# hiimmuc/SpeakerVerification

Hardware: AMD Instinct MI355X
Metric: embeddings/sec (2 s @16 kHz) (higher is better)
Workload: dtype bf16

## Files before the change

### speakerverification_amd/csrc/api_ecapa.hip

```cpp
#include <algorithm>

#include "handle.h"

namespace svhip {

namespace {

struct EcapaState : ModelState {
    ConvLayer blocks0, mfa, asp_tdnn, asp_conv;
    ConvLayer tdnn1[3], tdnn2[3], res2[3][7];
    LinearLayer se1[3], se2[3], asp_ctx, fc;
    float* se2T[3] = {};
    void *se1_bf[3] = {}, *se2T_bf[3] = {};
    float *aspbn_scale = nullptr, *aspbn_shift = nullptr;

    bool xin_ready = false;
    bool x0_is_s32 = false;
    bool cat_f32_stale = false;
    bool h2_is_s32 = false;
    bool h1_split = false;
    void* cat_s32 = nullptr;
    void* h2_s32 = nullptr;
    void* u_s32[2] = {};
    void* X0 = nullptr;
// ... 31 lines not shown
    auto tdnn = [&](const std::string& p, int64_t cin, int64_t cout, int64_t k) {
        spec[p + ".conv.conv.weight"] = {cout, cin, k}; spec[p + ".conv.conv.bias"] = {cout};
        spec_bn(spec, p + ".norm.norm", cout);
    };
    if (c.input_norm) { spec["instance_norm.weight"] = {nm}; spec["instance_norm.bias"] = {nm}; }
    tdnn("blocks.0", nm, C, ECAPA_K[0]);
    for (int i = 1; i <= 3; ++i) {
        const std::string p = "blocks." + std::to_string(i);
        tdnn(p + ".tdnn1", C, C, 1);
        for (int j = 0; j < 7; ++j) tdnn(p + ".res2net_block.blocks." + std::to_string(j), C / 8, C / 8, ECAPA_K[i]);
        tdnn(p + ".tdnn2", C, C, 1);
        spec[p + ".se_block.conv1.conv.weight"] = {128, C, 1}; spec[p + ".se_block.conv1.conv.bias"] = {128};
        spec[p + ".se_block.conv2.conv.weight"] = {C, 128, 1}; spec[p + ".se_block.conv2.conv.bias"] = {C};
    }
    tdnn("mfa", C3, C3, 1);
    tdnn("asp.tdnn", 3 * C3, 128, 1);
    spec["asp.conv.conv.weight"] = {C3, 128, 1}; spec["asp.conv.conv.bias"] = {C3};
    spec_bn(spec, "asp_bn.norm", 2 * C3);
    spec["fc.conv.weight"] = {(int64_t)c.embed_dim, 2 * C3, 1}; spec["fc.conv.bias"] = {(int64_t)c.embed_dim};
}

static int make_tdnn(svhip_handle* h, ConvLayer& L, const std::string& p, int dil) {
    return make_conv(h, L, p + ".conv.conv.weight", p + ".conv.conv.bias", p + ".norm.norm", dil);
}

int ecapa_finalize(svhip_handle* h) {
    auto& s = S(h);
    const int C = h->cfg.channels, C3 = 3 * C;
    int rc;
    if ((rc = make_tdnn(h, s.blocks0, "blocks.0", ECAPA_D[0]))) return rc;
    for (int i = 1; i <= 3; ++i) {
        const std::string p = "blocks." + std::to_string(i);
        if ((rc = make_tdnn(h, s.tdnn1[i - 1], p + ".tdnn1", 1))) return rc;
        for (int j = 0; j < 7; ++j)
            if ((rc = make_tdnn(h, s.res2[i - 1][j], p + ".res2net_block.blocks." + std::to_string(j), ECAPA_D[i]))) return rc;
        if ((rc = make_tdnn(h, s.tdnn2[i - 1], p + ".tdnn2", 1))) return rc;
        if ((rc = make_linear(h, s.se1[i - 1], p + ".se_block.conv1.conv.weight", p + ".se_block.conv1.conv.bias"))) return rc;
        if ((rc = make_linear(h, s.se2[i - 1], p + ".se_block.conv2.conv.weight", p + ".se_block.conv2.conv.bias"))) return rc;
        {
            const HostTensor* w2 = getw(h, p + ".se_block.conv2.conv.weight");
            std::vector<float> t((size_t)128 * C);
            for (int c = 0; c < C; ++c)
                for (int n = 0; n < 128; ++n) t[(size_t)n * C + c] = w2->data[(size_t)c * 128 + n];
            if ((rc = dev_upload(h, &s.se2T[i - 1], t))) return rc;
            if (h->bf16) {
                const HostTensor* w1 = getw(h, p + ".se_block.conv1.conv.weight");
                if ((rc = upload_h16(h, w1->data, &s.se1_bf[i - 1])) || (rc = upload_h16(h, t, &s.se2T_bf[i - 1]))) return rc;
            }
        }
    }
    if ((rc = make_tdnn(h, s.mfa, "mfa", 1))) return rc;
    if ((rc = make_conv(h, s.asp_tdnn, "asp.tdnn.conv.conv.weight", "", "asp.tdnn.norm.norm", 1, 0, C3))) return rc;
    if ((rc = make_linear(h, s.asp_ctx, "asp.tdnn.conv.conv.weight", "asp.tdnn.conv.conv.bias", C3, 3 * C3))) return rc;
    if ((rc = make_conv(h, s.asp_conv, "asp.conv.conv.weight", "asp.conv.conv.bias", "", 1))) return rc;
    if ((rc = make_bn(h, "asp_bn.norm", 2 * C3, &s.aspbn_scale, &s.aspbn_shift))) return rc;
    if ((rc = make_linear(h, s.fc, "fc.conv.weight", "fc.conv.bias"))) return rc;
    if (h->cfg.input_norm) {
        const HostTensor *w = getw(h, "instance_norm.weight"), *b = getw(h, "instance_norm.bias");
        if (!w || !b) SV_FAIL(h, SVHIP_ERR_MISSING, "missing instance_norm tensors");
        if ((rc = dev_upload(h, &h->in_w, w->data))) return rc;
        if ((rc = dev_upload(h, &h->in_b, b->data))) return rc;
    }
    const double T = h->T;
    double f = T * s.blocks0.flops_per_row + T * s.mfa.flops_per_row + T * s.asp_conv.flops_per_row;
    f += T * 2.0 * 128 * (3.0 * C3);
    for (int i = 0; i < 3; ++i) {
        f += T * (s.tdnn1[i].flops_per_row + s.tdnn2[i].flops_per_row);
        for (int j = 0; j < 7; ++j) f += T * s.res2[i][j].flops_per_row;
// ... 149 lines not shown
                                    h->x3 ? h->d_status : nullptr, h->host_flag_dev, (b0_cv && xscale) ? 3.0e38f : 65504.0f);
         }))) return rc;
    if (b0_cv) {
        if (xscale && (rc = run(h, "in_scale", 0, [&]() {
                 return launch_in_scale(static_cast<const float*>(p.X_in), (int64_t)M * c.n_mels, reinterpret_cast<uint32_t*>(xscale + 4), xscale, p.st, L.cv_wscale);
             }))) return rc;
        if ((rc = run(h, "split_s32", 0, [&]() { return launch_split_s32(static_cast<const float*>(p.X_in), c.n_mels, h->s32_buf, M, L.cv_cin, p.st, L.cv_cin, c.n_mels, xscale); }))) return rc;
        if ((rc = run(h, "gemm_pw3cv", (double)M * L.flops_per_row, [&]() { return launch_gemm_pw3cv(q, p.st); }))) return rc;
        p.x0_s32 = q.y_s32 != 0;
    } else {
        GemmParams g = conv_params(h, L, p.X_in, c.n_mels, p.X0, C, M, T);
        g.act1 = ACT_GELU;
        if ((rc = conv_gemm(h, L, g))) return rc;
    }
    s.x0_is_s32 = p.x0_s32;
    p.xin = p.x0_s32 ? nullptr : p.X0;
    p.xin32 = p.x0_s32 ? p.X0 : nullptr;
    p.ldin = p.ldin32 = C;
    return SVHIP_OK;
}

static int ec_res2(EcPass& p, int i, EcRes2 route, bool tdnn1_side) {
    svhip_handle* h = p.h;
    auto& s = p.s;
    const int T = h->T, M = p.M, C = h->cfg.channels, C8 = C / 8, e = h->esz;
    const bool bf = h->bf16;
    int rc;
    if (route == RES2_CHAIN) {
        Res2Params rp;
        rp.H1 = p.H1; rp.H2 = p.H2; rp.ld = C; rp.T = T; rp.dil = s.res2[i][0].dil; rp.Kp = s.res2[i][0].Kp;
        rp.slices = h->opt.r2_slices >= 0 ? std::max(1, h->opt.r2_slices) : res2net_chain_slices(p.B, C, T, rp.dil, h->num_cu);
        double fl = 0;
        for (int j = 0; j < 7; ++j) {
            rp.W[j] = s.res2[i][j].W; rp.bias[j] = s.res2[i][j].bias;
            rp.scale[j] = s.res2[i][j].scale; rp.shift[j] = s.res2[i][j].shift;
            fl += (double)M * s.res2[i][j].flops_per_row;
        }
        return run(h, rp.slices > 1 ? "res2net_slices" : "res2net_chain", fl, [&]() { return launch_res2net_chain(rp, p.B, C, p.st); });
    }
    if (route == RES2_LAYERS) {
        if ((rc = run(h, "copy_cols", 0, [&]() { return launch_copy_cols(p.H1, C, p.H2, C, bf, M, C8, p.st); }))) return rc;
        for (int j = 1; j < 8; ++j) {
            GemmParams q = conv_params(h, s.res2[i][j - 1], off(p.H1, (size_t)j * C8, e), C, off(p.H2, (size_t)j * C8, e), C, M, T);
            q.act1 = ACT_RELU;
            q.A2 = j >= 2 ? off(p.H2, (size_t)(j - 1) * C8, e) : nullptr; q.lda2 = C;
            if ((rc = conv_gemm(h, s.res2[i][j - 1], q))) return rc;
        }
        return SVHIP_OK;
    }
    if (!tdnn1_side) {
        if ((rc = run(h, "split_s32", 0, [&]() { return launch_split_s32(static_cast<const float*>(p.H1), C, p.h2s, M, C8, p.st, C); }))) return rc;
        if ((rc = run(h, "split_s32", 0, [&]() { return launch_split_s32(static_cast<const float*>(p.H1) + C8, C, p.us[0], M, C8, p.st, C8); }))) return rc;
    }
    for (int j = 1; j < 8; ++j) {
        const GemmParams q = ec_r2_step_params(p, i, j);
        if ((rc = run(h, route == RES2_STEP ? "r2_step" : "gemm_pw3r2", (double)M * s.res2[i][j - 1].flops_per_row, [&]() {
                 return route == RES2_STEP ? launch_r2_step(q, p.st) : launch_gemm_pw3r2(q, p.st);
             }))) return rc;
    }
    return SVHIP_OK;
}

static int ec_block(EcPass& p, int i) {
    svhip_handle* h = p.h;
    auto& s = p.s;
    const int T = h->T, B = p.B, C = h->cfg.channels, C3 = 3 * C, C8 = C / 8, e = h->esz;
    const bool bf = h->bf16;
// ... 286 lines not shown
```

### speakerverification_amd/csrc/api_weights.hip

```cpp
#include <algorithm>
#include <cmath>
#include <cstring>

#include "handle.h"

namespace svhip {

static inline uint16_t f32_to_f16_rne(float f) {
    const _Float16 hv = static_cast<_Float16>(f);
    uint16_t u;
    memcpy(&u, &hv, 2);
    return u;
}

uint16_t f32_to_bf16_rne(float f) {
    uint32_t u;
    memcpy(&u, &f, 4);
    if ((u & 0x7fffffffu) > 0x7f800000u) return (uint16_t)((u >> 16) | 0x40);
    u += 0x7fffu + ((u >> 16) & 1u);
    return (uint16_t)(u >> 16);
}

uint32_t x3_split_word(float v) {
#ifdef SVHIP_X3_BF16
    const uint16_t hi = f32_to_bf16_rne(v);
    uint32_t hu = (uint32_t)hi << 16;
    float hf; memcpy(&hf, &hu, 4);
    return hu | f32_to_bf16_rne(v - hf);
#else
    const _Float16 h = static_cast<_Float16>(v);
    const _Float16 l = static_cast<_Float16>(v - static_cast<float>(h));
    uint16_t hb, lb;
    memcpy(&hb, &h, 2); memcpy(&lb, &l, 2);
    return ((uint32_t)hb << 16) | lb;
#endif
}

// ... 231 lines not shown
                    for (int k = 0; k < L.K; ++k) { const float a = std::fabs(packed[(size_t)n * L.Kp + k]); if (std::isfinite(a) && a > wmax) wmax = a; }
                float sw = 1.0f;
                if (wmax > 0.0f && !(wmax >= 0x1p-8f && wmax < 0x1p13f)) { int e2; (void)std::frexp(wmax, &e2); sw = std::ldexp(1.0f, 7 - e2); }
                L.cv_wscale = sw;
                std::vector<uint16_t> s32((size_t)N * kcv * 2, 0);
                for (int n = 0; n < N; ++n)
                    for (int t = 0; t < taps; ++t)
                        for (int c = 0; c < cin; ++c) {
                            const uint32_t wv = sw == 1.0f ? ws[(size_t)n * L.Kp + t * cin + c] : x3_split_word(packed[(size_t)n * L.Kp + t * cin + c] * sw);
                            const int k = t * ccv + c;
                            const size_t o = (size_t)n * kcv * 2 + (size_t)(k >> 5) * 64 + (k & 31);
                            s32[o] = (uint16_t)(wv >> 16);
                            s32[o + 32] = (uint16_t)(wv & 0xffffu);
                        }
                uint16_t* dcv;
                if ((rc = dev_upload(h, &dcv, s32))) return rc;
                L.Wcv = dcv; L.cv_cin = ccv; L.cv_Kp = kcv;
            }
        }
    }
    if (bias && (rc = dev_upload(h, &L.bias, *bias))) return rc;
    return SVHIP_OK;
}

int make_conv(svhip_handle* h, ConvLayer& L, const std::string& wname, const std::string& bname, const std::string& bnname, int dil,
              int c_lo, int c_hi, bool rn_s32) {
    const HostTensor *w, *b = nullptr;
    int rc;
    if ((rc = needw(h, wname, w)) || (!bname.empty() && (rc = needw(h, bname, b)))) return rc;
    if ((rc = make_conv(h, L, *w, b ? &b->data : nullptr, dil, c_lo, c_hi, rn_s32))) return rc;
    return bnname.empty() ? SVHIP_OK : make_bn(h, bnname, L.N, &L.scale, &L.shift);
}

int make_linear(svhip_handle* h, LinearLayer& L, const std::string& wname, const std::string& bname, int c_lo, int c_hi) {
    const HostTensor *w, *b = nullptr;
    int rc;
    if ((rc = needw(h, wname, w))) return rc;
    const int N = (int)w->shape[0], Kfull = (int)w->shape[1];
    if (c_hi < 0) c_hi = Kfull;
    L.N = N; L.K = c_hi - c_lo;
    std::vector<float> m((size_t)N * L.K);
    for (int n = 0; n < N; ++n)
        for (int k = 0; k < L.K; ++k) m[(size_t)n * L.K + k] = w->data[(size_t)n * Kfull + c_lo + k];
    if ((rc = dev_upload(h, &L.W, m))) return rc;
    if (!bname.empty() && ((rc = needw(h, bname, b)) || (rc = dev_upload(h, &L.bias, b->data)))) return rc;
    return SVHIP_OK;
}

int upload_f32(svhip_handle* h, const std::string& name, float** dst) {
    const HostTensor* t;
    int rc = needw(h, name, t);
    return rc ? rc : dev_upload(h, dst, t->data);
}

int upload_h16(svhip_handle* h, const std::vector<float>& m, void** dst) {
    std::vector<uint16_t> v(m.size());
    for (size_t i = 0; i < m.size(); ++i) v[i] = f32_to_bf16_rne(m[i]);
    uint16_t* d;
    int rc = dev_upload(h, &d, v);
    *dst = d;
    return rc;
}

int actbuf(svhip_handle* h, void** dst, size_t elems) {
    char* p = nullptr;
    int rc = dev_alloc(h, &p, elems * h->esz + 256);
// ... 34 lines not shown
```

### speakerverification_amd/csrc/handle.h

```cpp
#pragma once
#include "../../include/svhip.h"

#include <hip/hip_runtime.h>

#include <cstdio>
#include <initializer_list>
#include <map>
#include <memory>
#include <string>
#include <vector>

#include "common.h"
#include "kernels.h"

namespace svhip {

struct HostTensor {
    std::vector<float> data;
    std::vector<int64_t> shape;
    int64_t numel() const { int64_t n = 1; for (auto s : shape) n *= s; return n; }
};

struct ConvLayer {
    int N = 0, K = 0, Kp = 0, Np = 0, taps = 1, dil = 1, cin = 0;
    void* W = nullptr;
    void* Wsplit = nullptr;
    float cv_wscale = 1.0f;
    void* Wcv = nullptr;
    int cv_cin = 0, cv_Kp = 0;
    void* Ws32 = nullptr;
    float* bias = nullptr;
    float* scale = nullptr;
    float* shift = nullptr;
    double flops_per_row = 0;
};

struct LinearLayer {
    int N = 0, K = 0;
    float* W = nullptr;
    float* bias = nullptr;
};

struct ModelState { virtual ~ModelState() = default; };
struct TailedBuf { const char* base; size_t bytes; };

constexpr int RAG_LEVELS = 7;

struct ProfEntry { std::string name; double ms = 0; int64_t launches = 0; double flops = 0; };
struct PendingEvent { hipEvent_t e0, e1; int entry; };

}

struct svhip_handle {
    svhip_config cfg{};
    hipStream_t stream = nullptr;
    bool own_stream = false;
    hipStream_t cur = nullptr;
    hipStream_t lane_stream[4] = {nullptr, nullptr, nullptr, nullptr};
// ... 141 lines not shown
        pe.e1 = prof_event(h);
        (void)hipEventRecord(pe.e0, h->cur);
    }
    hipError_t e = launch();
    if (e != hipSuccess) SV_FAIL(h, SVHIP_ERR_HIP, "launch %s failed: %s", label, hipGetErrorString(e));
    if (prof) {
        (void)hipEventRecord(pe.e1, h->cur);
        h->prof_entries[pe.entry].launches += 1;
        h->prof_entries[pe.entry].flops += flops;
        h->ev_pending.push_back(pe);
        if (h->ev_pending.size() >= 8192) prof_collect(h);
    }
    return SVHIP_OK;
}

inline void* off(void* base, size_t elems, int esz) { return reinterpret_cast<char*>(base) + elems * esz; }
inline const void* off(const void* base, size_t elems, int esz) { return reinterpret_cast<const char*>(base) + elems * esz; }

using WeightSpec = std::map<std::string, std::vector<int64_t>>;
int build_fbank_tables(svhip_handle* h);
int alloc_workspace(svhip_handle* h);
uint16_t f32_to_bf16_rne(float f);
uint32_t x3_split_word(float v);
uint16_t to_h16(const svhip_handle* h, float f);
const HostTensor* getw(svhip_handle* h, const std::string& name);
int needw(svhip_handle* h, const std::string& name, const HostTensor*& t);
void spec_bn(WeightSpec& spec, const std::string& p, int64_t n);
int bn_fold(svhip_handle* h, const std::string& p, int n, std::vector<double>& s, std::vector<double>& t);
int make_bn(svhip_handle* h, const std::string& p, int n, float** scale, float** shift);
int make_conv(svhip_handle* h, ConvLayer& L, const HostTensor& w, const std::vector<float>* bias, int dil, int c_lo = 0, int c_hi = -1,
              bool rn_s32 = false);
int make_conv(svhip_handle* h, ConvLayer& L, const std::string& wname, const std::string& bname, const std::string& bnname, int dil,
              int c_lo = 0, int c_hi = -1, bool rn_s32 = false);
int make_linear(svhip_handle* h, LinearLayer& L, const std::string& wname, const std::string& bname, int c_lo = 0, int c_hi = -1);
int upload_f32(svhip_handle* h, const std::string& name, float** dst);
int upload_h16(svhip_handle* h, const std::vector<float>& m, void** dst);
int actbuf(svhip_handle* h, void** dst, size_t elems);

struct StageView { const void* src; size_t rows, cols, ld; bool f32; };
using CheckFn = int(const svhip_config& c, const char*& err);
using SpecFn = void(const svhip_config& c, WeightSpec& spec);
using HandleFn = int(svhip_handle* h);
using EmbedFn = int(svhip_handle* h, const float* in, int B);
using StageFn = int(svhip_handle* h, const std::string& name, bool fill, StageView& v);
using RaggedCheckFn = int(const svhip_config& c, const int32_t* lengths, int n, bool is_wave, std::string& err);
using RaggedEmbedFn = int(svhip_handle* h, const float* in, bool in_host, bool is_wave, const int64_t* in_off, const int32_t* lengths, int n);
struct ModelOps {
    int model;
    CheckFn* check;
    SpecFn* spec;
    HandleFn *finalize, *alloc;
    EmbedFn *embed_wave, *embed_feat;
    StageFn* stage;
    int max_lanes;
    const char* optional_prefix;
    RaggedCheckFn* ragged_check;
    RaggedEmbedFn* embed_ragged;
};
int unknown_stage(svhip_handle* h, const std::string& name);

struct KeptStages {
    struct Kept { void* buf = nullptr; size_t rows = 0, cols = 0; bool f32 = false; uint64_t epoch = 0; int utts = 0; bool packed = false; size_t cap = 0; };
    std::map<std::string, Kept> kept;
    uint64_t epoch = 0;
};
enum { KEEP_DT, KEEP_F32, KEEP_S32 };
// ... 63 lines not shown
```

### speakerverification_amd/csrc/kernels.h

```cpp
#pragma once
#include <hip/hip_runtime.h>
#include <stdint.h>

#include <atomic>

#include "common.h"

namespace svhip {

struct DeviceOnce {
    std::atomic<uint64_t> mask{0};
    bool done(int dev) const { return dev >= 0 && dev < 64 && ((mask.load(std::memory_order_acquire) >> dev) & 1u); }
    void mark(int dev) { if (dev >= 0 && dev < 64) mask.fetch_or(1ull << dev, std::memory_order_release); }
};
inline hipError_t set_max_dynamic_lds(DeviceOnce& once, const void* fn, int bytes) {
    int dev = -1;
    hipError_t e = hipGetDevice(&dev);
    if (e != hipSuccess) return e;
    if (once.done(dev)) return hipSuccess;
    e = hipFuncSetAttribute(fn, hipFuncAttributeMaxDynamicSharedMemorySize, bytes);
    if (e == hipSuccess) once.mark(dev);
    return e;
}

// ... 72 lines not shown
hipError_t launch_rn_step(const GemmParams& p, int mode, hipStream_t stream);
bool gemm_pw3cv_supported(const GemmParams& p);
hipError_t launch_gemm_pw3cv(const GemmParams& p, hipStream_t stream);
bool gemm_n128_supported(const GemmParams& p);
hipError_t launch_gemm_n128(const GemmParams& p, hipStream_t stream);
bool gemm_pw3cv16_supported(const GemmParams& p);
hipError_t launch_gemm_pw3cv16(const GemmParams& p, hipStream_t stream);
bool gemm_pw3r2_supported(const GemmParams& p);
hipError_t launch_gemm_pw3r2(const GemmParams& p, hipStream_t stream);
hipError_t launch_split_s32(const float* src, int ld, void* dst, int64_t M, int K, hipStream_t stream, int ldd = 0, int kvalid = 0,
                            const float* scale = nullptr);
hipError_t launch_in_scale(const float* X, int64_t n, uint32_t* part256, float* scale, hipStream_t stream, float wscale = 1.0f);
hipError_t launch_unsplit_s32(const void* src, int lds32, float* dst, int ld, int64_t M, int K, hipStream_t stream);
int gemm_colsum_groups(const GemmParams& p, bool bf16);
hipError_t launch_gemm_ragged(const GemmParams& p, bool bf16, hipStream_t stream);

hipError_t launch_rag_rows(const int* row0, int n, int maxT, int* utt, hipStream_t stream);
hipError_t launch_rag_prologue(const float* feat, const int64_t* feat_off, const int* row0, int n, int maxT, void* out, bool out_bf16,
                               int n_mels, int log_input, const float* in_w, const float* in_b, float* stats, hipStream_t stream);
hipError_t launch_rag_colstats(const void* X, bool bf16, int ldx, const int* row0, int n, int C, float* out, bool with_std, float eps,
                               hipStream_t stream);
hipError_t launch_rag_se_apply(const void* h, int ldh, const float* s, const void* x, int ldx, void* out, int ldo, bool bf16,
                               const int* utt, int M, int C, hipStream_t stream);
hipError_t launch_rag_asp_pool(const float* logits, const void* X, bool bf16, int ldx, const int* row0, int n, int C, const float* bn_scale,
                               const float* bn_shift, float* pooled_raw, float* pooled_bn, float eps, hipStream_t stream, float var_max = 0.0f);
hipError_t launch_rag_linear(const float* in, int ld_in, const float* W, const float* bias, float* out, int ld_out, int n, int N, int K,
                             int act, hipStream_t stream);

struct Res2Params {
    const void* H1 = nullptr;
    void* H2 = nullptr;
    int ld = 0, T = 0, dil = 1, Kp = 0;
    const void* W[7] = {};
    const float* bias[7] = {};
    const float* scale[7] = {};
    const float* shift[7] = {};
    int debug = 0;
    unsigned long long* ts = nullptr;
    int slices = 1;
    int Tc = 0;
};
bool res2net_chain_supported(int C, int T, int dil, int Kp);
int res2net_chain_slices(int B, int C, int T, int dil, int num_cu);
hipError_t launch_res2net_chain(const Res2Params& p, int B, int C, hipStream_t stream);

struct FbankTables {
    const float* basis = nullptr;
    const void* basis_hi = nullptr;
    const void* basis_lo = nullptr;
    const void* basis_l3 = nullptr;
    const void* sym_hi = nullptr;
    const void* sym_lo = nullptr;
    int split6 = 0;
    int n_k16 = 13;
    int split_bf16 = 0;
    const float* mel_w = nullptr;
    int n_melw = 0;
    const int* mel_start = nullptr;
    const int* mel_len = nullptr;
    const int* mel_off = nullptr;
    int n_fft = 512, win_length = 200, hop = 80, n_mels = 80, n_bins = 257, lpad = 156;
    int n_pairs = 9;
    int n_q = 25;
    int mel_max_bin = 256;
    int force32 = 0;
    float preemph = 0.97f;
// ... 290 lines not shown
```

### speakerverification_amd/csrc/res2net.hip

```cpp
#include "common.h"
#include "kernels.h"

namespace svhip {

namespace {

#ifdef SVHIP_GEMM_DEBUG
constexpr bool R2DBG = true;
#else
constexpr bool R2DBG = false;
#endif
constexpr int R2_TMAX = 416;

template <int CW, int MIT> struct R2Cfg {
    static constexpr int ROWB = CW * 2;
    static constexpr int NCH = ROWB / 16;
    static constexpr int NT = CW / 32;
    static constexpr int MW = 8 / NT;
    static constexpr int MI = MIT;
    static constexpr int TMAX = MW * MI * 32 < R2_TMAX ? MW * MI * 32 : R2_TMAX;
    static constexpr int U_BYTES = TMAX * ROWB;
    static constexpr int W_BYTES = CW * ROWB;
    static constexpr int LDS = U_BYTES + W_BYTES;
    static constexpr int WCH = CW * NCH / 512;
    static __device__ __forceinline__ int swz(int row) { return CW == 128 ? (row & 15) : ((row >> 1) & 7); }
};

template <int CW, int MIT>
__global__ __launch_bounds__(512, 2) void res2net_chain_kernel(Res2Params p) {
    typedef R2Cfg<CW, MIT> CF;
    constexpr int ROWB = CF::ROWB, NCH = CF::NCH, MI = CF::MI, WCH = CF::WCH;
    extern __shared__ __attribute__((aligned(16))) char smem[];
    char* U = smem;
    char* Wt = smem + CF::U_BYTES;

    const int S = p.slices > 1 ? p.slices : 1;
    const int b = (int)blockIdx.x / S, si = (int)blockIdx.x - b * S;
    const int Tg = p.T;
    const int c0 = S > 1 ? si * p.Tc : 0, c1 = S > 1 ? min(Tg, c0 + p.Tc) : Tg;
    const int l0 = S > 1 ? max(0, c0 - 7 * p.dil) : 0, l1 = S > 1 ? min(Tg, c1 + 7 * p.dil) : Tg;
    const int T = l1 - l0;
    const int tid = threadIdx.x, lane = tid & 63;
    const int wave = __builtin_amdgcn_readfirstlane(tid >> 6);
    const int wn = wave % CF::NT, wq = wave / CF::NT;
    const int fr = lane & 31, fh = lane >> 5;
    const bf16_t* __restrict__ H1 = reinterpret_cast<const bf16_t*>(p.H1) + ((int64_t)b * Tg + l0) * p.ld;
    bf16_t* __restrict__ H2 = reinterpret_cast<bf16_t*>(p.H2) + ((int64_t)b * Tg + l0) * p.ld;
    const int s0 = c0 - l0, s1 = c1 - l0;

    u32x4 wregs[WCH];
    auto wload = [&](int layer, int tap) {
        const char* wsrc = reinterpret_cast<const char*>(p.W[layer]);
        int tid_w = tid;
        asm volatile("" : "+v"(tid_w));
#pragma unroll
        for (int e = 0; e < WCH; ++e) {
            const int c = tid_w + 512 * e;
            const int n = c / NCH, ch = c % NCH;
            wregs[e] = *reinterpret_cast<const u32x4*>(wsrc + ((int64_t)n * p.Kp + tap * CW) * 2 + ch * 16);
        }
    };
    auto wstore = [&]() {
        int tid_w = tid;
        asm volatile("" : "+v"(tid_w));
#pragma unroll
        for (int e = 0; e < WCH; ++e) {
            const int c = tid_w + 512 * e;
            const int n = c / NCH, ch = c % NCH;
            *reinterpret_cast<u32x4*>(Wt + n * ROWB + ((ch ^ CF::swz(n)) << 4)) = wregs[e];
        }
    };

    wload(0, 0);
    {
        constexpr int RSTEP = 512 / NCH, RB0 = 4;
        const int row0 = tid / NCH, ch0 = tid % NCH;
        const uint32_t goff0 = ((uint32_t)row0 * (uint32_t)p.ld + (uint32_t)ch0 * 8u) * 2u;
        const uint32_t gstep = (uint32_t)RSTEP * (uint32_t)p.ld * 2u;
        const char* h1b = reinterpret_cast<const char*>(H1);
        char* h2b = reinterpret_cast<char*>(H2);
        for (int it0 = 0; it0 * RSTEP < T; it0 += RB0) {
            u32x4 cc0[RB0], cc1[RB0];
#pragma unroll
            for (int k = 0; k < RB0; ++k)
                if (row0 + (it0 + k) * RSTEP < T) {
                    cc0[k] = __builtin_nontemporal_load(reinterpret_cast<const u32x4*>(h1b + goff0 + (uint32_t)(it0 + k) * gstep));
                    cc1[k] = __builtin_nontemporal_load(reinterpret_cast<const u32x4*>(h1b + CW * 2 + goff0 + (uint32_t)(it0 + k) * gstep));
                }
#pragma unroll
            for (int k = 0; k < RB0; ++k) {
                const int row = row0 + (it0 + k) * RSTEP;
                if (row < T) {
                    if (row >= s0 && row < s1) *reinterpret_cast<u32x4*>(h2b + goff0 + (uint32_t)(it0 + k) * gstep) = cc0[k];
                    *reinterpret_cast<u32x4*>(U + row * ROWB + ((ch0 ^ CF::swz(row)) << 4)) = cc1[k];
                }
            }
        }
    }
    wstore();
    __syncthreads();
    const bool stamp = R2DBG && (p.debug & 64) && p.ts && tid == 0;
    unsigned long long tprev = 0;
    if (R2DBG && (p.debug & 64) && p.ts) tprev = __builtin_readcyclecounter();
    if (stamp) p.ts[(size_t)blockIdx.x * 32 + 3] = tprev;
#define R2_STAMP(stage, k) if (R2DBG && (p.debug & 64) && p.ts) { const unsigned long long t_ = __builtin_readcyclecounter(); if (stamp) p.ts[(size_t)blockIdx.x * 32 + (stage) * 4 + (k)] = t_ - tprev; tprev = t_; }

    for (int s = 1; s < 8; ++s) {
        const int layer = s - 1;
        f32x16 acc[MI];
        float zero = 0.0f;
        asm volatile("" : "+v"(zero));
#pragma unroll
        for (int i = 0; i < MI; ++i)
#pragma unroll
            for (int r = 0; r < 16; ++r) acc[i][r] = zero;

        constexpr int RSTEP = 512 / NCH;
        constexpr int RB = 7;
        constexpr int NPRE = (CF::TMAX / RSTEP + RB - 1) / RB * RB;
        const bool noglob = R2DBG && (p.debug & 1);

        u32x4 cpre[NPRE];
        for (int tap = 0; tap < 3; ++tap) {
            if (tap == 2 && s < 7 && !noglob) {
                int tid_p = tid;
                asm volatile("" : "+v"(tid_p));
                const int row0 = tid_p / NCH, ch0 = tid_p % NCH;
                const char* h1s = reinterpret_cast<const char*>(H1) + (s + 1) * CW * 2;
#pragma unroll
                for (int k = 0; k < NPRE; ++k) {
                    const int rowc = min(row0 + k * RSTEP, T - 1);
                    cpre[k] = __builtin_nontemporal_load(reinterpret_cast<const u32x4*>(h1s + ((uint32_t)rowc * (uint32_t)p.ld + (uint32_t)ch0 * 8u) * 2u));
                }
            }
            const bool more = !(s == 7 && tap == 2);
            if (more && !(R2DBG && (p.debug & 4))) { if (tap < 2) wload(layer, tap + 1); else wload(layer + 1, 0); }
            const int delta = (tap - 1) * p.dil;
            int fh_t = fh, fr_t = fr;
            asm volatile("" : "+v"(fh_t), "+v"(fr_t));
            int rbase[MI], rsw[MI];
#pragma unroll
            for (int i = 0; i < MI; ++i) {
                const int t = (wq + CF::MW * i) * 32 + fr_t + delta;
                const int row = min(max(reflect_idx(l0 + t, Tg) - l0, 0), T - 1);
                rbase[i] = row * ROWB;
                rsw[i] = CF::swz(row);
            }
            const int wrow = (wn * 32 + fr_t);
            const int wbase = wrow * ROWB, wsw = CF::swz(wrow);
            if (!(R2DBG && (p.debug & 2))) {
                constexpr int NK = CW / 16;
#pragma unroll
                for (int kk = 0; kk < NK; ++kk) {
                    const int ch = 2 * kk + fh_t;
                    const bf16x8 wf = *reinterpret_cast<const bf16x8*>(Wt + wbase + ((ch ^ wsw) << 4));
                    bf16x8 xf[MI];
#pragma unroll
                    for (int i = 0; i < MI; ++i) xf[i] = *reinterpret_cast<const bf16x8*>(U + rbase[i] + ((ch ^ rsw[i]) << 4));
#pragma unroll
                    for (int i = 0; i < MI; ++i) acc[i] = __builtin_amdgcn_mfma_f32_32x32x16_bf16(wf, xf[i], acc[i], 0, 0, 0);
                }
            }
            __syncthreads();
            if (tap < 2) { if (!(R2DBG && (p.debug & 4))) wstore(); __syncthreads(); }
        }

        R2_STAMP(s, 0)
        int fh_e = fh, fr_e = fr;
        asm volatile("" : "+v"(fh_e), "+v"(fr_e));
        if (!(R2DBG && (p.debug & 8)))
#pragma unroll
        for (int g = 0; g < 4; ++g) {
            const int n = wn * 32 + 8 * g + 4 * fh_e;
            const f32x4 b4 = *reinterpret_cast<const f32x4*>(p.bias[layer] + n);
            const f32x4 sc4 = *reinterpret_cast<const f32x4*>(p.scale[layer] + n);
            const f32x4 sh4 = *reinterpret_cast<const f32x4*>(p.shift[layer] + n);
#pragma unroll
            for (int i = 0; i < MI; ++i) {
                const int t = (wq + CF::MW * i) * 32 + fr_e;
                if (t < T) {
                    typedef bf16_t bf16x4 __attribute__((ext_vector_type(4)));
                    bf16x4 o;
#pragma unroll
                    for (int e = 0; e < 4; ++e) o[e] = static_cast<bf16_t>(fmaf(fmaxf(acc[i][4 * g + e] + b4[e], 0.0f), sc4[e], sh4[e]));
                    const int c8 = n >> 2;
                    *reinterpret_cast<bf16x4*>(U + t * ROWB + ((((c8 >> 1) ^ CF::swz(t)) << 4) | ((c8 & 1) << 3))) = o;
                }
            }
        }
        if (s < 7 && !(R2DBG && (p.debug & 4))) wstore();
        __syncthreads();
        R2_STAMP(s, 1)

        if (R2DBG && (p.debug & 32)) {
            for (int c = tid; c < T * NCH; c += 512) {
                const int row = c / NCH, ch = c % NCH;
                char* up = U + row * ROWB + ((ch ^ CF::swz(row)) << 4);
                const bf16x8 y = *reinterpret_cast<const bf16x8*>(up);
                if (row >= s0 && row < s1) *reinterpret_cast<bf16x8*>(H2 + (int64_t)row * p.ld + s * CW + ch * 8) = y;
                if (s < 7) {
                    const bf16x8 cn = *reinterpret_cast<const bf16x8*>(H1 + (int64_t)row * p.ld + (s + 1) * CW + ch * 8);
                    bf16x8 u;
#pragma unroll
                    for (int e = 0; e < 8; ++e) u[e] = static_cast<bf16_t>(static_cast<float>(y[e]) + static_cast<float>(cn[e]));
                    *reinterpret_cast<bf16x8*>(up) = u;
                }
            }
        } else {
            int tid_r = tid;
            asm volatile("" : "+v"(tid_r));
            const int row0 = tid_r / NCH, ch0 = tid_r % NCH;
            const uint32_t goff0 = ((uint32_t)row0 * (uint32_t)p.ld + (uint32_t)ch0 * 8u) * 2u;
            const uint32_t gstep = (uint32_t)RSTEP * (uint32_t)p.ld * 2u;
            char* h2s = reinterpret_cast<char*>(H2) + s * CW * 2;
#pragma unroll
            for (int g = 0; g < NPRE / RB; ++g) {
                const int it0 = g * RB;
                if (it0 * RSTEP < T) {
#pragma unroll
                    for (int k = 0; k < RB; ++k) {
                        const int row = row0 + (it0 + k) * RSTEP;
                        if (row < T) {
                            char* up = U + row * ROWB + ((ch0 ^ CF::swz(row)) << 4);
                            const bf16x8 y = *reinterpret_cast<const bf16x8*>(up);
                            if (!noglob && row >= s0 && row < s1) *reinterpret_cast<bf16x8*>(h2s + goff0 + (uint32_t)(it0 + k) * gstep) = y;
                            if (s < 7 && !noglob) {
                                const bf16x8 cv = __builtin_bit_cast(bf16x8, cpre[it0 + k]);
                                bf16x8 u;
#pragma unroll
                                for (int e = 0; e < 8; ++e) u[e] = static_cast<bf16_t>(static_cast<float>(y[e]) + static_cast<float>(cv[e]));
                                *reinterpret_cast<bf16x8*>(up) = u;
                            }
                        }
                    }
                }
            }
        }
        __syncthreads();
        R2_STAMP(s, 2)
    }
#undef R2_STAMP
}

template <int CW, int MIT>
hipError_t launch_cw(const Res2Params& p, int grid, hipStream_t stream) {
    static DeviceOnce attr;
    constexpr int lds = R2Cfg<CW, MIT>::LDS;
    if (hipError_t e = set_max_dynamic_lds(attr, reinterpret_cast<const void*>(res2net_chain_kernel<CW, MIT>), lds)) return e;
    hipLaunchKernelGGL((res2net_chain_kernel<CW, MIT>), dim3(grid), dim3(512), lds, stream, p);
    return hipGetLastError();
}

}

int res2net_chain_slices(int B, int C, int T, int dil, int num_cu) {
    const int cw = C / 8;
    const int tmax_s = cw == 128 ? R2Cfg<128, 3>::TMAX : R2Cfg<64, 2>::TMAX;
    int best = 1;
    for (int S = 2; S <= 7; ++S) {
        const int tc = (T + S - 1) / S;
        if ((int64_t)S * B > (int64_t)num_cu) break;
        if (tc + 14 * dil <= tmax_s && tc > 14 * dil) best = S;
    }
    return best;
}

bool res2net_chain_supported(int C, int T, int dil, int Kp) {
    const int cw = C / 8;
    return (cw == 64 || cw == 128) && T <= R2_TMAX && T > 2 * dil && Kp == 3 * cw;
}

hipError_t launch_res2net_chain(const Res2Params& p_in, int B, int C, hipStream_t stream) {
    if (!res2net_chain_supported(C, p_in.T, p_in.dil, p_in.Kp) || B <= 0 || p_in.ld % 8 != 0) return hipErrorInvalidValue;
    Res2Params p = p_in;
    if (p.slices > 1) {
        const int tmax_s = C / 8 == 128 ? R2Cfg<128, 3>::TMAX : R2Cfg<64, 2>::TMAX;
        while (p.slices > 1) {
            p.Tc = (p.T + p.slices - 1) / p.slices;
            if (p.Tc + 14 * p.dil <= tmax_s && p.Tc > 14 * p.dil) break;
            --p.slices;
        }
        if (p.slices > 1) return C / 8 == 128 ? launch_cw<128, 3>(p, B * p.slices, stream) : launch_cw<64, 2>(p, B * p.slices, stream);
    }
    p.slices = 1;
    return C / 8 == 128 ? launch_cw<128, 7>(p, B, stream) : launch_cw<64, 4>(p, B, stream);
}

}
```

Before: 57880.

## Prepack res2net weights into MFMA fragments and stream them straight into registers

Res2Net conv weights are repacked on the host into MFMA-fragment order, so each lane loads its B fragment from global memory directly into registers. This replaces the old scheme of staging them through LDS with extra barriers per tap. Weight prefetch for the next tap or layer now overlaps with the MFMAs of the current one, using scheduling barriers. Bias, scale and shift for all seven layers are cached in LDS once, and the stage loop is split so the last stage is specialised at compile time. The cost is higher register pressure and more global weight traffic per wave, and the path now requires packed weights to be present.

```diff
diff --git a/speakerverification_amd/csrc/api_ecapa.hip b/speakerverification_amd/csrc/api_ecapa.hip
--- a/speakerverification_amd/csrc/api_ecapa.hip
+++ b/speakerverification_amd/csrc/api_ecapa.hip
@@ -87,8 +87,10 @@
     for (int i = 1; i <= 3; ++i) {
         const std::string p = "blocks." + std::to_string(i);
         if ((rc = make_tdnn(h, s.tdnn1[i - 1], p + ".tdnn1", 1))) return rc;
-        for (int j = 0; j < 7; ++j)
-            if ((rc = make_tdnn(h, s.res2[i - 1][j], p + ".res2net_block.blocks." + std::to_string(j), ECAPA_D[i]))) return rc;
+        for (int j = 0; j < 7; ++j) {
+            const std::string q = p + ".res2net_block.blocks." + std::to_string(j);
+            if ((rc = make_tdnn(h, s.res2[i - 1][j], q, ECAPA_D[i])) || (rc = make_res2_wf(h, s.res2[i - 1][j], q + ".conv.conv.weight"))) return rc;
+        }
         if ((rc = make_tdnn(h, s.tdnn2[i - 1], p + ".tdnn2", 1))) return rc;
         if ((rc = make_linear(h, s.se1[i - 1], p + ".se_block.conv1.conv.weight", p + ".se_block.conv1.conv.bias"))) return rc;
         if ((rc = make_linear(h, s.se2[i - 1], p + ".se_block.conv2.conv.weight", p + ".se_block.conv2.conv.bias"))) return rc;
@@ -304,7 +306,7 @@
         rp.slices = h->opt.r2_slices >= 0 ? std::max(1, h->opt.r2_slices) : res2net_chain_slices(p.B, C, T, rp.dil, h->num_cu);
         double fl = 0;
         for (int j = 0; j < 7; ++j) {
-            rp.W[j] = s.res2[i][j].W; rp.bias[j] = s.res2[i][j].bias;
+            rp.W[j] = s.res2[i][j].W; rp.Wf[j] = s.res2[i][j].Wf; rp.bias[j] = s.res2[i][j].bias;
             rp.scale[j] = s.res2[i][j].scale; rp.shift[j] = s.res2[i][j].shift;
             fl += (double)M * s.res2[i][j].flops_per_row;
         }
diff --git a/speakerverification_amd/csrc/api_weights.hip b/speakerverification_amd/csrc/api_weights.hip
--- a/speakerverification_amd/csrc/api_weights.hip
+++ b/speakerverification_amd/csrc/api_weights.hip
@@ -3,6 +3,7 @@
 #include <cstring>
 
 #include "handle.h"
+#include "res2_pack.h"
 
 namespace svhip {
 
@@ -300,6 +301,23 @@
     return bnname.empty() ? SVHIP_OK : make_bn(h, bnname, L.N, &L.scale, &L.shift);
 }
 
+int make_res2_wf(svhip_handle* h, ConvLayer& L, const std::string& wname) {
+    if (!h->bf16 || !res2_wf_supported(L.cin, L.N, L.cin, L.taps, L.Kp)) return SVHIP_OK;
+    const HostTensor* w;
+    int rc;
+    if ((rc = needw(h, wname, w))) return rc;
+    const int cw = L.cin;
+    std::vector<uint16_t> pb((size_t)cw * L.Kp), pf(res2_wf_elems(cw));
+    for (int n = 0; n < cw; ++n)
+        for (int t = 0; t < 3; ++t)
+            for (int c = 0; c < cw; ++c) pb[(size_t)n * L.Kp + t * cw + c] = to_h16(h, w->data[((size_t)n * cw + c) * 3 + t]);
+    res2_pack_wf(pb.data(), L.Kp, cw, pf.data());
+    uint16_t* d;
+    if ((rc = dev_upload(h, &d, pf))) return rc;
+    L.Wf = d;
+    return SVHIP_OK;
+}
+
 int make_linear(svhip_handle* h, LinearLayer& L, const std::string& wname, const std::string& bname, int c_lo, int c_hi) {
     const HostTensor *w, *b = nullptr;
     int rc;
diff --git a/speakerverification_amd/csrc/handle.h b/speakerverification_amd/csrc/handle.h
--- a/speakerverification_amd/csrc/handle.h
+++ b/speakerverification_amd/csrc/handle.h
@@ -24,6 +24,7 @@
 struct ConvLayer {
     int N = 0, K = 0, Kp = 0, Np = 0, taps = 1, dil = 1, cin = 0;
     void* W = nullptr;
+    void* Wf = nullptr;
     void* Wsplit = nullptr;
     float cv_wscale = 1.0f;
     void* Wcv = nullptr;
@@ -231,6 +232,7 @@
               bool rn_s32 = false);
 int make_conv(svhip_handle* h, ConvLayer& L, const std::string& wname, const std::string& bname, const std::string& bnname, int dil,
               int c_lo = 0, int c_hi = -1, bool rn_s32 = false);
+int make_res2_wf(svhip_handle* h, ConvLayer& L, const std::string& wname);
 int make_linear(svhip_handle* h, LinearLayer& L, const std::string& wname, const std::string& bname, int c_lo = 0, int c_hi = -1);
 int upload_f32(svhip_handle* h, const std::string& name, float** dst);
 int upload_h16(svhip_handle* h, const std::vector<float>& m, void** dst);
diff --git a/speakerverification_amd/csrc/kernels.h b/speakerverification_amd/csrc/kernels.h
--- a/speakerverification_amd/csrc/kernels.h
+++ b/speakerverification_amd/csrc/kernels.h
@@ -128,6 +128,7 @@
     void* H2 = nullptr;
     int ld = 0, T = 0, dil = 1, Kp = 0;
     const void* W[7] = {};
+    const void* Wf[7] = {};
     const float* bias[7] = {};
     const float* scale[7] = {};
     const float* shift[7] = {};
diff --git a/speakerverification_amd/csrc/res2_pack.h b/speakerverification_amd/csrc/res2_pack.h
--- /dev/null
+++ b/speakerverification_amd/csrc/res2_pack.h
@@ -0,0 +1,29 @@
+#pragma once
+#include <cstddef>
+#include <cstdint>
+
+namespace svhip {
+
+constexpr int RES2_WF_FRAG_BYTES = 1024;
+
+constexpr bool res2_wf_supported(int cw, int N, int cin, int taps, int Kp) {
+    return (cw == 64 || cw == 128) && N == cw && cin == cw && taps == 3 && Kp == 3 * cw;
+}
+
+constexpr size_t res2_wf_elems(int cw) { return (size_t)3 * cw * cw; }
+
+constexpr size_t res2_wf_frag_offset(int cw, int tap, int wn, int kk) {
+    return (((size_t)tap * (cw / 32) + wn) * (cw / 16) + kk) * RES2_WF_FRAG_BYTES;
+}
+
+constexpr size_t res2_wf_index(int cw, int tap, int n, int k) {
+    return res2_wf_frag_offset(cw, tap, n >> 5, k >> 4) / 2 + (size_t)((((k >> 3) & 1) << 5) | (n & 31)) * 8 + (k & 7);
+}
+
+inline void res2_pack_wf(const uint16_t* W, int Kp, int cw, uint16_t* Wf) {
+    for (int tap = 0; tap < 3; ++tap)
+        for (int n = 0; n < cw; ++n)
+            for (int k = 0; k < cw; ++k) Wf[res2_wf_index(cw, tap, n, k)] = W[(size_t)n * Kp + tap * cw + k];
+}
+
+}
diff --git a/speakerverification_amd/csrc/res2net.hip b/speakerverification_amd/csrc/res2net.hip
--- a/speakerverification_amd/csrc/res2net.hip
+++ b/speakerverification_amd/csrc/res2net.hip
@@ -1,5 +1,7 @@
+#include <type_traits>
 #include "common.h"
 #include "kernels.h"
+#include "res2_pack.h"
 
 namespace svhip {
 
@@ -20,19 +22,24 @@
     static constexpr int MI = MIT;
     static constexpr int TMAX = MW * MI * 32 < R2_TMAX ? MW * MI * 32 : R2_TMAX;
     static constexpr int U_BYTES = TMAX * ROWB;
-    static constexpr int W_BYTES = CW * ROWB;
-    static constexpr int LDS = U_BYTES + W_BYTES;
-    static constexpr int WCH = CW * NCH / 512;
+    static constexpr int NK = CW / 16;
+    static constexpr int V_BYTES = 21 * CW * 4;
+    static constexpr int TS_BYTES = R2DBG ? 32 * 8 : 0;
+    static constexpr int LDS = U_BYTES + V_BYTES + TS_BYTES;
     static __device__ __forceinline__ int swz(int row) { return CW == 128 ? (row & 15) : ((row >> 1) & 7); }
 };
 
-template <int CW, int MIT>
+constexpr int R2_VMCNT0 = 0x0F70;
+constexpr int R2_SCHED_KEEP_MFMA_VMEM = 0x0002 | 0x0004 | 0x0080 | 0x0100 | 0x0200;
+
+template <int CW, int MIT, int DBG>
 __global__ __launch_bounds__(512, 2) void res2net_chain_kernel(Res2Params p) {
     typedef R2Cfg<CW, MIT> CF;
-    constexpr int ROWB = CF::ROWB, NCH = CF::NCH, MI = CF::MI, WCH = CF::WCH;
+    constexpr int ROWB = CF::ROWB, NCH = CF::NCH, MI = CF::MI, NK = CF::NK;
+    constexpr bool noglob = DBG & 1, nomfma = DBG & 2, noweights = DBG & 4, noepi = DBG & 8, plainrows = DBG & 32;
     extern __shared__ __attribute__((aligned(16))) char smem[];
     char* U = smem;
-    char* Wt = smem + CF::U_BYTES;
+    float* V = reinterpret_cast<float*>(smem + CF::U_BYTES);
 
     const int S = p.slices > 1 ? p.slices : 1;
     const int b = (int)blockIdx.x / S, si = (int)blockIdx.x - b * S;
@@ -48,30 +55,24 @@
     bf16_t* __restrict__ H2 = reinterpret_cast<bf16_t*>(p.H2) + ((int64_t)b * Tg + l0) * p.ld;
     const int s0 = c0 - l0, s1 = c1 - l0;
 
-    u32x4 wregs[WCH];
-    auto wload = [&](int layer, int tap) {
-        const char* wsrc = reinterpret_cast<const char*>(p.W[layer]);
-        int tid_w = tid;
-        asm volatile("" : "+v"(tid_w));
-#pragma unroll
-        for (int e = 0; e < WCH; ++e) {
-            const int c = tid_w + 512 * e;
-            const int n = c / NCH, ch = c % NCH;
-            wregs[e] = *reinterpret_cast<const u32x4*>(wsrc + ((int64_t)n * p.Kp + tap * CW) * 2 + ch * 16);
-        }
+    bf16x8 wf[NK];
+    auto wfrag = [&](const void* wl, int tap, int kk) {
+        return *reinterpret_cast<const bf16x8*>(reinterpret_cast<const char*>(wl) + res2_wf_frag_offset(CW, tap, wn, kk) + (uint32_t)lane * 16u);
     };
-    auto wstore = [&]() {
-        int tid_w = tid;
-        asm volatile("" : "+v"(tid_w));
-#pragma unroll
-        for (int e = 0; e < WCH; ++e) {
-            const int c = tid_w + 512 * e;
-            const int n = c / NCH, ch = c % NCH;
-            *reinterpret_cast<u32x4*>(Wt + n * ROWB + ((ch ^ CF::swz(n)) << 4)) = wregs[e];
-        }
-    };
-
-    wload(0, 0);
+#pragma unroll
+    for (int kk = 0; kk < NK; ++kk) wf[kk] = wfrag(p.Wf[0], 0, kk);
+
+    if (tid < 3 * CW) {
+        const int which = tid / CW, n = tid - which * CW;
+        float v[7];
+#pragma unroll
+        for (int l = 0; l < 7; ++l) v[l] = (which == 0 ? p.bias[l] : which == 1 ? p.scale[l] : p.shift[l])[n];
+#pragma unroll
+        for (int l = 0; l < 7; ++l) V[(l * 3 + which) * CW + n] = v[l];
+    }
+#pragma unroll
+    for (int kk = 0; kk < NK; ++kk) asm volatile("" : "+v"(wf[kk]));
+
     {
         constexpr int RSTEP = 512 / NCH, RB0 = 4;
         const int row0 = tid / NCH, ch0 = tid % NCH;
@@ -87,6 +88,7 @@
                     cc0[k] = __builtin_nontemporal_load(reinterpret_cast<const u32x4*>(h1b + goff0 + (uint32_t)(it0 + k) * gstep));
                     cc1[k] = __builtin_nontemporal_load(reinterpret_cast<const u32x4*>(h1b + CW * 2 + goff0 + (uint32_t)(it0 + k) * gstep));
                 }
+            __builtin_amdgcn_s_waitcnt(R2_VMCNT0);
 #pragma unroll
             for (int k = 0; k < RB0; ++k) {
                 const int row = row0 + (it0 + k) * RSTEP;
@@ -97,15 +99,17 @@
             }
         }
     }
-    wstore();
     __syncthreads();
-    const bool stamp = R2DBG && (p.debug & 64) && p.ts && tid == 0;
+    constexpr bool STAMPS = R2DBG && (DBG & 64);
+    unsigned long long* tsl = reinterpret_cast<unsigned long long*>(smem + CF::U_BYTES + CF::V_BYTES);
+    const bool stamp = STAMPS && p.ts && tid == 0;
     unsigned long long tprev = 0;
-    if (R2DBG && (p.debug & 64) && p.ts) tprev = __builtin_readcyclecounter();
-    if (stamp) p.ts[(size_t)blockIdx.x * 32 + 3] = tprev;
-#define R2_STAMP(stage, k) if (R2DBG && (p.debug & 64) && p.ts) { const unsigned long long t_ = __builtin_readcyclecounter(); if (stamp) p.ts[(size_t)blockIdx.x * 32 + (stage) * 4 + (k)] = t_ - tprev; tprev = t_; }
-
-    for (int s = 1; s < 8; ++s) {
+    if (STAMPS && p.ts) tprev = __builtin_readcyclecounter();
+    if (stamp) tsl[3] = tprev;
+#define R2_STAMP(stage, k) if (STAMPS && p.ts) { const unsigned long long t_ = __builtin_readcyclecounter(); if (stamp) tsl[(stage) * 4 + (k)] = t_ - tprev; tprev = t_; }
+
+    auto stage = [&](const int s, auto last_tag) __attribute__((always_inline)) {
+        constexpr bool LAST = decltype(last_tag)::value;
         const int layer = s - 1;
         f32x16 acc[MI];
         float zero = 0.0f;
@@ -118,23 +122,29 @@
         constexpr int RSTEP = 512 / NCH;
         constexpr int RB = 7;
         constexpr int NPRE = (CF::TMAX / RSTEP + RB - 1) / RB * RB;
-        const bool noglob = R2DBG && (p.debug & 1);
+        const void* wcur = p.Wf[layer];
+        const void* wnxt = p.Wf[LAST ? layer : layer + 1];
 
         u32x4 cpre[NPRE];
+#pragma unroll
         for (int tap = 0; tap < 3; ++tap) {
-            if (tap == 2 && s < 7 && !noglob) {
-                int tid_p = tid;
-                asm volatile("" : "+v"(tid_p));
-                const int row0 = tid_p / NCH, ch0 = tid_p % NCH;
-                const char* h1s = reinterpret_cast<const char*>(H1) + (s + 1) * CW * 2;
-#pragma unroll
-                for (int k = 0; k < NPRE; ++k) {
-                    const int rowc = min(row0 + k * RSTEP, T - 1);
-                    cpre[k] = __builtin_nontemporal_load(reinterpret_cast<const u32x4*>(h1s + ((uint32_t)rowc * (uint32_t)p.ld + (uint32_t)ch0 * 8u) * 2u));
-                }
-            }
-            const bool more = !(s == 7 && tap == 2);
-            if (more && !(R2DBG && (p.debug & 4))) { if (tap < 2) wload(layer, tap + 1); else wload(layer + 1, 0); }
+            if (tap == 2 && !LAST) {
+                __builtin_amdgcn_sched_barrier(0);
+                if (!noglob) {
+                    int tid_p = tid;
+                    asm volatile("" : "+v"(tid_p));
+                    const int row0 = tid_p / NCH, ch0 = tid_p % NCH;
+                    const char* h1s = reinterpret_cast<const char*>(H1) + (s + 1) * CW * 2;
+#pragma unroll
+                    for (int k = 0; k < NPRE; ++k) {
+                        const int rowc = min(row0 + k * RSTEP, T - 1);
+                        cpre[k] = __builtin_nontemporal_load(reinterpret_cast<const u32x4*>(h1s + ((uint32_t)rowc * (uint32_t)p.ld + (uint32_t)ch0 * 8u) * 2u));
+                    }
+                }
+                __builtin_amdgcn_sched_barrier(0);
+            }
+            const bool refill = !noweights && (tap < 2 || !LAST);
+            const void* wsrc = tap < 2 ? wcur : wnxt;
             const int delta = (tap - 1) * p.dil;
             int fh_t = fh, fr_t = fr;
             asm volatile("" : "+v"(fh_t), "+v"(fr_t));
@@ -146,35 +156,35 @@
                 rbase[i] = row * ROWB;
                 rsw[i] = CF::swz(row);
             }
-            const int wrow = (wn * 32 + fr_t);
-            const int wbase = wrow * ROWB, wsw = CF::swz(wrow);
-            if (!(R2DBG && (p.debug & 2))) {
-                constexpr int NK = CW / 16;
-#pragma unroll
-                for (int kk = 0; kk < NK; ++kk) {
-                    const int ch = 2 * kk + fh_t;
-                    const bf16x8 wf = *reinterpret_cast<const bf16x8*>(Wt + wbase + ((ch ^ wsw) << 4));
+#pragma unroll
+            for (int kk = 0; kk < NK; ++kk) {
+                const int ch = 2 * kk + fh_t;
+                if (!nomfma) {
                     bf16x8 xf[MI];
 #pragma unroll
                     for (int i = 0; i < MI; ++i) xf[i] = *reinterpret_cast<const bf16x8*>(U + rbase[i] + ((ch ^ rsw[i]) << 4));
 #pragma unroll
-                    for (int i = 0; i < MI; ++i) acc[i] = __builtin_amdgcn_mfma_f32_32x32x16_bf16(wf, xf[i], acc[i], 0, 0, 0);
-                }
-            }
-            __syncthreads();
-            if (tap < 2) { if (!(R2DBG && (p.debug & 4))) wstore(); __syncthreads(); }
-        }
+                    for (int i = 0; i < MI; ++i) acc[i] = __builtin_amdgcn_mfma_f32_32x32x16_bf16(wf[kk], xf[i], acc[i], 0, 0, 0);
+                }
+                if (refill) {
+                    wf[kk] = wfrag(wsrc, tap < 2 ? tap + 1 : 0, kk);
+                    __builtin_amdgcn_sched_barrier(R2_SCHED_KEEP_MFMA_VMEM);
+                }
+            }
+        }
+        __syncthreads();
 
         R2_STAMP(s, 0)
         int fh_e = fh, fr_e = fr;
         asm volatile("" : "+v"(fh_e), "+v"(fr_e));
-        if (!(R2DBG && (p.debug & 8)))
+        if (!noepi)
 #pragma unroll
         for (int g = 0; g < 4; ++g) {
             const int n = wn * 32 + 8 * g + 4 * fh_e;
-            const f32x4 b4 = *reinterpret_cast<const f32x4*>(p.bias[layer] + n);
-            const f32x4 sc4 = *reinterpret_cast<const f32x4*>(p.scale[layer] + n);
-            const f32x4 sh4 = *reinterpret_cast<const f32x4*>(p.shift[layer] + n);
+            const float* vl = V + layer * 3 * CW + n;
+            const f32x4 b4 = *reinterpret_cast<const f32x4*>(vl);
+            const f32x4 sc4 = *reinterpret_cast<const f32x4*>(vl + CW);
+            const f32x4 sh4 = *reinterpret_cast<const f32x4*>(vl + 2 * CW);
 #pragma unroll
             for (int i = 0; i < MI; ++i) {
                 const int t = (wq + CF::MW * i) * 32 + fr_e;
@@ -188,17 +198,16 @@
                 }
             }
         }
-        if (s < 7 && !(R2DBG && (p.debug & 4))) wstore();
         __syncthreads();
         R2_STAMP(s, 1)
 
-        if (R2DBG && (p.debug & 32)) {
+        if (plainrows) {
             for (int c = tid; c < T * NCH; c += 512) {
                 const int row = c / NCH, ch = c % NCH;
                 char* up = U + row * ROWB + ((ch ^ CF::swz(row)) << 4);
                 const bf16x8 y = *reinterpret_cast<const bf16x8*>(up);
                 if (row >= s0 && row < s1) *reinterpret_cast<bf16x8*>(H2 + (int64_t)row * p.ld + s * CW + ch * 8) = y;
-                if (s < 7) {
+                if (!LAST) {
                     const bf16x8 cn = *reinterpret_cast<const bf16x8*>(H1 + (int64_t)row * p.ld + (s + 1) * CW + ch * 8);
                     bf16x8 u;
 #pragma unroll
@@ -207,6 +216,7 @@
                 }
             }
         } else {
+            if (!LAST) __builtin_amdgcn_s_waitcnt(R2_VMCNT0);
             int tid_r = tid;
             asm volatile("" : "+v"(tid_r));
             const int row0 = tid_r / NCH, ch0 = tid_r % NCH;
@@ -224,7 +234,7 @@
                             char* up = U + row * ROWB + ((ch0 ^ CF::swz(row)) << 4);
                             const bf16x8 y = *reinterpret_cast<const bf16x8*>(up);
                             if (!noglob && row >= s0 && row < s1) *reinterpret_cast<bf16x8*>(h2s + goff0 + (uint32_t)(it0 + k) * gstep) = y;
-                            if (s < 7 && !noglob) {
+                            if (!LAST && !noglob) {
                                 const bf16x8 cv = __builtin_bit_cast(bf16x8, cpre[it0 + k]);
                                 bf16x8 u;
 #pragma unroll
@@ -238,17 +248,37 @@
         }
         __syncthreads();
         R2_STAMP(s, 2)
-    }
+    };
+    for (int s = 1; s < 7; ++s) stage(s, std::false_type{});
+    stage(7, std::true_type{});
 #undef R2_STAMP
+    if (STAMPS && p.ts && tid < 32) p.ts[(size_t)blockIdx.x * 32 + tid] = tsl[tid];
+}
+
+template <int CW, int MIT, int DBG>
+hipError_t launch_dbg(const Res2Params& p, int grid, hipStream_t stream) {
+    static DeviceOnce attr;
+    constexpr int lds = R2Cfg<CW, MIT>::LDS;
+    if (hipError_t e = set_max_dynamic_lds(attr, reinterpret_cast<const void*>(res2net_chain_kernel<CW, MIT, DBG>), lds)) return e;
+    hipLaunchKernelGGL((res2net_chain_kernel<CW, MIT, DBG>), dim3(grid), dim3(512), lds, stream, p);
+    return hipGetLastError();
 }
 
 template <int CW, int MIT>
 hipError_t launch_cw(const Res2Params& p, int grid, hipStream_t stream) {
-    static DeviceOnce attr;
-    constexpr int lds = R2Cfg<CW, MIT>::LDS;
-    if (hipError_t e = set_max_dynamic_lds(attr, reinterpret_cast<const void*>(res2net_chain_kernel<CW, MIT>), lds)) return e;
-    hipLaunchKernelGGL((res2net_chain_kernel<CW, MIT>), dim3(grid), dim3(512), lds, stream, p);
-    return hipGetLastError();
+#ifdef SVHIP_GEMM_DEBUG
+    switch (p.debug) {
+        case 0: break;
+        case 1: return launch_dbg<CW, MIT, 1>(p, grid, stream);
+        case 2: return launch_dbg<CW, MIT, 2>(p, grid, stream);
+        case 4: return launch_dbg<CW, MIT, 4>(p, grid, stream);
+        case 8: return launch_dbg<CW, MIT, 8>(p, grid, stream);
+        case 32: return launch_dbg<CW, MIT, 32>(p, grid, stream);
+        case 64: return launch_dbg<CW, MIT, 64>(p, grid, stream);
+        default: return hipErrorInvalidValue;
+    }
+#endif
+    return launch_dbg<CW, MIT, 0>(p, grid, stream);
 }
 
 }
@@ -272,6 +302,8 @@
 
 hipError_t launch_res2net_chain(const Res2Params& p_in, int B, int C, hipStream_t stream) {
     if (!res2net_chain_supported(C, p_in.T, p_in.dil, p_in.Kp) || B <= 0 || p_in.ld % 8 != 0) return hipErrorInvalidValue;
+    for (int j = 0; j < 7; ++j)
+        if (!p_in.Wf[j] || !p_in.bias[j] || !p_in.scale[j] || !p_in.shift[j]) return hipErrorInvalidValue;
     Res2Params p = p_in;
     if (p.slices > 1) {
         const int tmax_s = C / 8 == 128 ? R2Cfg<128, 3>::TMAX : R2Cfg<64, 2>::TMAX;
```

Measured after the change: 58460, median of 6. 1.01x the previous value.
